# timsu1104/Open-vocabulary-3D-Object-Detection

Hardware: AMD Instinct MI355X
Metric: scenes/sec (train step) SUN RGB-D 20k pts nqueries=128 (higher is better)
Workload: dtype bf16; 1 GPU; SUN RGB-D train step, bs=8/GPU, 20000 pts, nqueries=128, 3DETR 256-d enc3/dec8, text-emb 640, AdamW + clip 0.1; global_batch=8, points=20000, parallelism=dp1

## Files before the change

include/ov3d.h:

```cpp
#ifndef OV3D_H_
#define OV3D_H_

#include <stdint.h>

#ifdef __cplusplus
extern "C" {
#endif

#define OV3D_OK 0
#define OV3D_EINVAL (-1)
#define OV3D_ELAUNCH (-2)

const char* ov3d_version(void);

int ov3d_fps(const float* xyz, int B, int N, int M, int32_t* idx_out, float* new_xyz_out,
             float* workspace, void* stream);
long long ov3d_fps_workspace(int B, int N);
int ov3d_fps_pair_status(const float* workspace, int B, int N, int M, int32_t* status,
                         void* stream);

int ov3d_nbr_max_fwd(const void* y, long long P, int S, int C, void* out, uint8_t* arg,
                     void* stream);
int ov3d_nbr_max_bwd(const void* g, const uint8_t* arg, long long P, int S, int C, void* dy,
                     void* stream);
// ... 234 lines not shown
                      const float* be2, float eps, const void* W1, long long ldw1, const void* b1,
                      float pf, int site_ffn, const void* W2, long long ldw2, const void* b2,
                      int k_quarters, float* s1, float* mean, float* rstd, void* x2, void* h,
                      void* y2, void* stream);
int ov3d_enc_post_bwd(int R, const float* ds1, const void* dy2, const float* s1, const float* mean,
                      const float* rstd, const void* h, const float* g2, const void* Wo,
                      long long ldwo, const void* W1, long long ldw1, const void* W2,
                      long long ldw2, float p1, const int64_t* seed, int site1, float pf,
                      int k_quarters, float* ds, void* dy1, void* dout, void* d1, float* partials,
                      int nparts, void* stream);

int ov3d_attn_fwd(const void* q, const void* k, const void* v, long long sq, long long sk,
                  long long sv, int B, int H, int Lq, int Lk, float scale, float dropout_p,
                  const int64_t* seed, int site, void* o, long long so, float* lse,
                  uint32_t* dropbits, float* workspace, int nsplit, void* stream);
long long ov3d_attn_fwd_workspace(int B, int H, int Lq, int Lk, int nsplit);
long long ov3d_attn_dropbits_words(int B, int H, int Lq, int Lk);
int ov3d_attn_bwd(const void* q, const void* k, const void* v, long long sq, long long sk,
                  long long sv, const void* o, long long so, const void* dout, long long sdo,
                  const float* lse, int B, int H, int Lq, int Lk, float scale, float dropout_p,
                  const uint32_t* dropbits, float* dvec, void* dq, long long sdq, void* dk,
                  long long sdk, void* dv, long long sdv, float* workspace, int nsplit,
                  void* stream);

typedef struct {
    const void* q; long long sq; const void* k; long long sk; const void* v; long long sv;
    const void* dout; long long sdo; const float* lse; const float* dvec;
    const uint32_t* dropbits; void* dk; long long sdk; void* dv; long long sdv;
} ov3d_attn_dkdv_job;
int ov3d_attn_bwd_dkdv_batch(const ov3d_attn_dkdv_job* jobs, int njobs, int B, int H, int Lq,
                             int Lk, float scale, float dropout_p, void* stream);

int ov3d_attn_small_bwd(int on);

long long ov3d_attn_maskbits_words(int B, int Lq, int Lk);
int ov3d_attn_mask_pack(const void* src, int kind, float thr, int B, int Lq, int Lk,
                        uint32_t* words, void* stream);
int ov3d_attn_fwd_masked(const void* q, const void* k, const void* v, long long sq, long long sk,
                         long long sv, int B, int H, int Lq, int Lk, float scale, float dropout_p,
                         const int64_t* seed, int site, void* o, long long so, float* lse,
                         uint32_t* dropbits, float* workspace, int nsplit,
                         const uint32_t* maskbits, void* stream);
int ov3d_attn_fwd_pregen(const void* q, const void* k, const void* v, long long sq, long long sk,
                         long long sv, int B, int H, int Lq, int Lk, float scale, float dropout_p,
                         const int64_t* seed, int site, void* o, long long so, float* lse,
                         uint32_t* dropbits, float* workspace, int nsplit, const uint32_t* maskbits,
                         void* stream);
int ov3d_attn_dropgen(int B, int H, int Lq, int Lk, float dropout_p, const int64_t* seed, int site,
                      uint32_t* dropbits, void* stream);
int ov3d_attn_bwd_masked(const void* q, const void* k, const void* v, long long sq, long long sk,
                         long long sv, const void* o, long long so, const void* dout, long long sdo,
                         const float* lse, int B, int H, int Lq, int Lk, float scale,
                         float dropout_p, const uint32_t* dropbits, float* dvec, void* dq,
                         long long sdq, void* dk, long long sdk, void* dv, long long sdv,
                         float* workspace, int nsplit, const uint32_t* maskbits, void* stream);

int ov3d_wgrad(const void* dy, long long ldy, const void* x, long long ldx, int R, int N, int K,
               float* dW, long long ldw, float* db, float* workspace, int* counters, int nsplit,
               void* stream);
int ov3d_wgrad_bn(const void* dy, long long ldy, const void* x, long long ldx, int R, int N, int K,
                  const float* scale, const float* shift, float* dW, long long ldw, float* db,
                  float* workspace, int* counters, int nsplit, void* stream);
long long ov3d_wgrad_workspace(int R, int N, int K, int nsplit);
typedef struct {
    const void* dy; long long ldy; const void* x; long long ldx;
    int R, N, K, nsplit;
// ... 277 lines not shown
```

open-vocabulary-3d-object-detection_amd/csrc/attn.hip:

```cpp
#include <math.h>
#include <type_traits>
#include <stdlib.h>

#include "common.h"

namespace {

typedef __bf16 bf16;
typedef __bf16 bf16x8 __attribute__((ext_vector_type(8)));
typedef __bf16 bf16x4 __attribute__((ext_vector_type(4)));
typedef float f32x16 __attribute__((ext_vector_type(16)));
typedef short s16x4 __attribute__((ext_vector_type(4)));
typedef float f32x2 __attribute__((ext_vector_type(2)));
typedef __bf16 bf16x2 __attribute__((ext_vector_type(2)));
typedef uint32_t u32x4 __attribute__((ext_vector_type(4)));
typedef short s16x2 __attribute__((ext_vector_type(2)));

constexpr int D = 64;
constexpr int KB = 64;
constexpr int QW = 32;
constexpr int LDK = 72;

__device__ __forceinline__ int isw(int r) { return (((r >> 1) & 1) << 2) | ((r >> 2) & 3); }
__device__ __forceinline__ int img(int r, int c) { return r * D + 8 * ((c >> 3) ^ isw(r)) + (c & 7); }
// ... 96 lines not shown
    return fmaxf(__builtin_bit_cast(float, (uint32_t)r[0]), __builtin_bit_cast(float, (uint32_t)r[1]));
}

__device__ __forceinline__ bf16x8 prescale8(bf16x8 v, float c) {
    bf16x8 r;
#pragma unroll
    for (int j = 0; j < 8; ++j) r[j] = (bf16)((float)v[j] * c);
    return r;
}

__device__ __forceinline__ bf16x8 kslots(float x0, float x1, bool on) {
    bf16x8 r;
#pragma unroll
    for (int j = 0; j < 8; ++j) r[j] = (bf16)0.f;
    if (on) {
        r[0] = (bf16)x0;
        r[1] = (bf16)x1;
    }
    return r;
}
__device__ __forceinline__ float bf16_hi(float x) { return (float)(bf16)x; }
__device__ __forceinline__ float bf16_lo(float x) {
    return __builtin_isinf(x) ? 0.f : x - bf16_hi(x);
}

constexpr float kStabBig = 32768.f;
__device__ __forceinline__ float stabiliser(float x) {
    const float hi = bf16_hi(x);
    return fabsf(x) < kStabBig ? hi : hi + bf16_hi(bf16_lo(x));
}

constexpr float RESCALE_THR = 8.f;

constexpr int kMaxCombine = 16;

#ifdef OV3D_ATTN_PROBE
__device__ unsigned long long* g_attn_probe;
#define PROBE_ENTRY const unsigned long long pr_entry = __builtin_amdgcn_s_memtime();
#define PROBE_DECL unsigned long long pr_t = __builtin_amdgcn_s_memtime(), pr_acc[8] = {0, 0, 0, 0, 0, 0, 0, 0}; \
    pr_acc[7] = pr_t - pr_entry;
#define PROBE(i) do { const unsigned long long t_ = __builtin_amdgcn_s_memtime(); pr_acc[i] += t_ - pr_t; pr_t = t_; } while (0)
#define PROBE_END do { if ((threadIdx.x & 63) == 0 && g_attn_probe) { \
    unsigned long long* o_ = g_attn_probe + (((size_t)blockIdx.z * gridDim.y + blockIdx.y) * gridDim.x + blockIdx.x) * 32 + (threadIdx.x >> 6) * 8; \
    for (int i_ = 0; i_ < 8; ++i_) o_[i_] = pr_acc[i_]; } } while (0)
#else
#define PROBE_ENTRY
#define PROBE_DECL
#define PROBE(i) do { } while (0)
#define PROBE_END do { } while (0)
#endif

__device__ __forceinline__ f32x16 mfma(bf16x8 a, bf16x8 b, f32x16 c) {
    return __builtin_amdgcn_mfma_f32_32x32x16_bf16(a, b, c, 0, 0, 0);
}

__device__ __forceinline__ bf16x4 tr16(const bf16* p) {
    s16x4 r = __builtin_amdgcn_ds_read_tr16_b64_v4i16(
        (__attribute__((address_space(3))) s16x4*)(p));
    return __builtin_bit_cast(bf16x4, r);
}

__device__ __forceinline__ bf16x8 v_operand(const bf16* Vs, int lane, int dt, int t, int s) {
    const int g = lane >> 4, i = lane & 15;
    const int d0 = 32 * dt + 16 * (g & 1) + 4 * (i & 3);
    const int k0 = 32 * t + 16 * s + 4 * (g >> 1) + (i >> 2);
    const bf16x4 lo = tr16(Vs + img(k0, d0));
// ... 36 lines not shown
    const int tid = threadIdx.x, lane = tid & 63, wave = tid >> 6;
    const int r = lane & 31, h = lane >> 5;
    int bx, bh;
    xcd_block(bx, bh);
    const int q0 = bx * (4 * QW) + wave * QW;
    if (q0 >= a.Lq) return;
    const uint32_t qh = drop_query_base(drop_head_mix(a.seed, a.site, bh), q0 + r) +
                        (uint32_t)(2 * h) * kPairMul;
    uint32_t* const wq_lane = a.wq + ((size_t)bh * a.Lq + q0 + r) * 2 + h;
    const size_t wq_tile = (size_t)gridDim.y * a.Lq * 2;
    uint32_t* const wk_lane = a.wk + ((size_t)(q0 >> 5) * gridDim.y + bh) * ((size_t)a.nkt * 64) +
                              drop_key(r, h);
    const short ts = (short)((int)a.thresh - 32768);
    const s16x2 tsig = {ts, ts};
    const int per = (a.nkt + gridDim.z - 1) / gridDim.z;
    const int kt1 = min(a.nkt, (int)(blockIdx.z + 1) * per);
    for (int kt = blockIdx.z * per; kt < kt1; ++kt) {
        const uint32_t hb = qh + (uint32_t)(32 * kt) * kPairMul;
        uint32_t dw = 0;
#pragma unroll
        for (int t = 0; t < 2; ++t)
#pragma unroll
            for (int i = 0; i < 16; i += 2) {
                const uint32_t c = 16 * t + ((i & 3) >> 1) + 4 * (i >> 2);
                const uint32_t dm = drop_halves(drop_mix(hb + c * kPairMul), tsig);
                const int jb = 8 * t + (i >> 1);
                dw |= dm & ((1u << jb) | (1u << (16 + jb)));
            }
        wq_lane[(size_t)kt * wq_tile] = dw;
        wk_lane[64 * kt] = transpose32(dw, r);
    }
}

template <bool DROP, bool MASK, bool BITS>
__device__ __forceinline__ void attn_fwd_body(const AttnArgs& a) {
    PROBE_ENTRY
    __shared__ __attribute__((aligned(16))) bf16 KVs[2][2][KB * LDK];
    bf16 (*const Ks)[KB * LDK] = KVs[0];
    bf16 (*const Vs)[KB * LDK] = KVs[1];
    const int tid = threadIdx.x, lane = tid & 63, wave = tid >> 6;
    const int r = lane & 31, h = lane >> 5;
    int bx, bh;
    xcd_block(bx, bh);
    const int b = bh / a.H, hh = bh - b * a.H;
    const int q0 = bx * (4 * QW) + wave * QW;
    const bool active = q0 < a.Lq;
    const int kbeg = blockIdx.z * a.keys_per_split;
    const int kend = min(a.Lk, kbeg + a.keys_per_split);

    bf16x8 qf[4];
    {
        const int qi = active ? q0 + r : 0;
        const bf16* qrow = a.q + ((size_t)qi * a.B + b) * a.sq + hh * D;
#pragma unroll
        for (int s = 0; s < 4; ++s)
            qf[s] = prescale8(*reinterpret_cast<const bf16x8*>(qrow + 16 * s + 8 * h), a.scale2);
    }
    uint32_t qh = 0;
    if (DROP && !BITS) qh = drop_query_base(drop_head_mix(a.seed, a.site, bh), active ? q0 + r : 0) +
                            (uint32_t)(2 * h) * kPairMul;
    uint32_t* const wq_lane = DROP ? a.wq + ((size_t)bh * a.Lq + (active ? q0 + r : 0)) * 2 + h : nullptr;
    const size_t wq_tile = (size_t)gridDim.y * a.Lq * 2;
    uint32_t* const wk_lane = (DROP && !BITS) ? a.wk + ((size_t)(q0 >> 5) * gridDim.y + bh) * ((size_t)a.nkt * 64) +
                                         drop_key(r, h) : nullptr;
    uint32_t dw_prev = 0;
    uint32_t dw_cur = 0, dw_next = 0;
    uint32_t mw_cur = 0, mw_next = 0;
    const uint32_t* const mrow = MASK ? a.mq + ((size_t)b * a.Lq + (active ? q0 + r : 0)) * 2 + h : nullptr;
    const size_t mtile = (size_t)a.B * a.Lq * 2;
    auto store_drop = [&](int kbp) {
        wq_lane[(size_t)(kbp >> 6) * wq_tile] = dw_prev;
        wk_lane[kbp] = transpose32(dw_prev, r);
// ... 17 lines not shown
            const int key = kb + (tid >> 3) + 32 * c;
            size_t ko = k0off + (size_t)(kb + 32 * c) * rowk, vo = v0off + (size_t)(kb + 32 * c) * rowv;
            if (key >= a.Lk) {
                ko -= (size_t)(key - (a.Lk - 1)) * rowk;
                vo -= (size_t)(key - (a.Lk - 1)) * rowv;
            }
            kr[c] = *reinterpret_cast<const bf16x8*>(a.k + ko);
            vr[c] = *reinterpret_cast<const bf16x8*>(a.v + vo);
        }
    };
    auto store = [&](int buf) {
#pragma unroll
        for (int c = 0; c < 2; ++c) {
            const int idx = tid + 256 * c, key = idx >> 3, ch = idx & 7;
            *reinterpret_cast<bf16x8*>(&Ks[buf][img(key, 8 * ch)]) = kr[c];
            *reinterpret_cast<bf16x8*>(&Vs[buf][img(key, 8 * ch)]) = vr[c];
        }
    };

    f32x16 o[2];
#pragma unroll
    for (int i = 0; i < 16; ++i) o[0][i] = o[1][i] = 0.f;
    float mb = 0.f;
    bool unset = true;
    const bf16x8 k1 = kslots(1.f, 1.f, h == 0);
    bf16x8 kmb = kslots(0.f, 0.f, false);
    f32x16 lacc;
#pragma unroll
    for (int i = 0; i < 16; ++i) lacc[i] = 0.f;
    bf16x8 ones;
#pragma unroll
    for (int j = 0; j < 8; ++j) ones[j] = (bf16)1.f;

    if (kbeg < kend) {
        load(kbeg);
        store(0);
        if (DROP && BITS && active) dw_cur = wq_lane[(size_t)(kbeg >> 6) * wq_tile];
        if (MASK && active) mw_cur = mrow[(size_t)(kbeg >> 6) * mtile];
    }
    __syncthreads();
    PROBE_DECL
    int buf = 0;
    for (int kb = kbeg; kb < kend; kb += KB, buf ^= 1) {
        const bool more = kb + KB < kend;
        PROBE(0);
        {
            const bf16* K = Ks[buf];
            const bf16* V = Vs[buf];
            if (MASK && more) mw_next = mrow[(size_t)((kb >> 6) + 1) * mtile];
            const uint32_t mw = mw_cur;
            if (DROP && BITS && more) dw_next = wq_lane[(size_t)((kb >> 6) + 1) * wq_tile];
            const uint32_t kwin = ~dw_cur;
            bf16x8 ka[2][4];
#pragma unroll
            for (int t = 0; t < 2; ++t)
#pragma unroll
                for (int s = 0; s < 4; ++s)
                    ka[t][s] = *reinterpret_cast<const bf16x8*>(K + img(32 * t + r, 16 * s + 8 * h));
            f32x16 st[2];
#pragma unroll
            for (int t = 0; t < 2; ++t) {
#pragma unroll
                for (int i = 0; i < 16; ++i)
                    st[t][i] = MASK ? __builtin_bit_cast(float, bit_mask(mw, score_bit(t, i)) & 0xFF800000u) : 0.f;
                st[t] = mfma(k1, kmb, st[t]);
            }
#pragma unroll
            for (int s = 0; s < 4; ++s)
#pragma unroll
                for (int t = 0; t < 2; ++t) st[t] = mfma(ka[t][s], qf[s], st[t]);
            bf16x8 va[2][2][2];
#pragma unroll
            for (int dt = 0; dt < 2; ++dt)
#pragma unroll
                for (int t = 0; t < 2; ++t)
#pragma unroll
                    for (int s = 0; s < 2; ++s) va[dt][t][s] = v_operand(V, lane, dt, t, s);
            if (more) load(kb + KB);
            if (DROP && !BITS && kb > kbeg && active) store_drop(kb - KB);
            PROBE(1);
            const int nvalid = kend - kb;
            if (nvalid < KB) {
#pragma unroll
                for (int t = 0; t < 2; ++t)
#pragma unroll
                    for (int i = 0; i < 16; ++i)
                        if (32 * t + (i & 3) + 8 * (i >> 2) + 4 * h >= nvalid) st[t][i] = -INFINITY;
            }
            float mx = -INFINITY;
#pragma unroll
            for (int t = 0; t < 2; ++t)
#pragma unroll
                for (int i = 0; i < 16; ++i) mx = fmaxf(mx, st[t][i]);
            mx = max_halves(mx);
            PROBE(2);
            const bool seen = mx > -INFINITY;
            if (__any(mx > RESCALE_THR || (unset && seen))) {
                const float mn = (mx > 0.f || (unset && seen)) ? stabiliser(mb + mx) : mb;
                const float d = mn - mb;
                const float alpha = unset ? 1.f : fast_exp2(-d);
                lacc[0] *= alpha;
#pragma unroll
                for (int i = 0; i < 16; ++i) {
                    o[0][i] *= alpha;
                    o[1][i] *= alpha;
                }
#pragma unroll
                for (int t = 0; t < 2; ++t)
#pragma unroll
                    for (int i = 0; i < 16; ++i) st[t][i] -= d;
                mb = mn;
// ... 16 lines not shown
#endif
                    uint32_t pk = pack_bf16(p0, p1);
                    praw[t][i >> 3][(i & 7) >> 1] = pk;
                    if (DROP && BITS) {
                        const int jb = 8 * t + (i >> 1);
                        const s16x2 kh = __builtin_bit_cast(s16x2, kwin << (15 - jb));
                        pk &= __builtin_bit_cast(uint32_t, (s16x2)(kh >> (s16x2){15, 15}));
                    } else if (DROP) {
                        const uint32_t c = 16 * t + ((i & 3) >> 1) + 4 * (i >> 2);
                        const uint32_t dm = drop_halves(drop_mix(hb + c * kPairMul), tsig);
                        pk &= ~dm;
                        const int jb = 8 * t + (i >> 1);
                        dw |= dm & ((1u << jb) | (1u << (16 + jb)));
                    }
                    pw[t][i >> 3][(i & 7) >> 1] = pk;
                }
            if (DROP && !BITS) dw_prev = dw;
            if (DROP && BITS) dw_cur = dw_next;
            if (MASK) mw_cur = mw_next;
            PROBE(3);
#pragma unroll
            for (int t = 0; t < 2; ++t)
#pragma unroll
                for (int s = 0; s < 2; ++s) {
                    const bf16x8 pf = __builtin_bit_cast(bf16x8, pw[t][s]);
#pragma unroll
                    for (int dt = 0; dt < 2; ++dt) o[dt] = mfma(va[dt][t][s], pf, o[dt]);
#ifndef OV3D_ATTN_VALU_ROWSUM
                    lacc = mfma(ones, __builtin_bit_cast(bf16x8, praw[t][s]), lacc);
#endif
                }
        }
        PROBE(4);
        if (more) store(buf ^ 1);
        PROBE(5);
        __syncthreads();
        PROBE(6);
    }
    PROBE_END;
    if (active && DROP && !BITS && kend > kbeg) store_drop((kend - 1) & ~(KB - 1));
#ifdef OV3D_ATTN_VALU_ROWSUM
    const float ltot = l + __shfl_xor(l, 32);
#else
    const float ltot = lacc[0];
#endif
    const int q = q0 + r;
    const int ql = wave * QW + r;
    if (a.nsplit == 1) {
        const float inv = ltot > 0.f ? a.keep_scale / ltot : 0.f;
        bf16* const so = &KVs[0][0][0];
#pragma unroll
        for (int dt = 0; dt < 2; ++dt)
#pragma unroll
            for (int g = 0; g < 4; ++g) {
                bf16x4 w;
#pragma unroll
                for (int j = 0; j < 4; ++j) w[j] = (bf16)(o[dt][4 * g + j] * inv);
                *reinterpret_cast<bf16x4*>(so + ql * LDK + 32 * dt + 8 * g + 4 * h) = w;
            }
        if (active && h == 0) a.lse[(size_t)bh * a.Lq + q] = mb + log2f(ltot);
        __syncthreads();
#pragma unroll
        for (int i = 0; i < 4; ++i) {
            const int c = tid + 256 * i, row = c >> 3, d8 = (c & 7) * 8;
            const int qq = bx * (4 * QW) + row;
            if (qq < a.Lq)
                *reinterpret_cast<bf16x8*>(a.o + ((size_t)qq * a.B + b) * a.so + hh * D + d8) =
                    *reinterpret_cast<const bf16x8*>(so + row * LDK + d8);
        }
    } else {
        constexpr int LDF = D + 4;
        float* const sf = reinterpret_cast<float*>(&KVs[0][0][0]);
        static_assert(sizeof(KVs) >= 128 * LDF * sizeof(float), "fp32 staging rows overrun KVs");
#pragma unroll
        for (int dt = 0; dt < 2; ++dt)
#pragma unroll
            for (int g = 0; g < 4; ++g)
                *reinterpret_cast<float4*>(sf + ql * LDF + 32 * dt + 8 * g + 4 * h) =
                    make_float4(o[dt][4 * g] * a.keep_scale, o[dt][4 * g + 1] * a.keep_scale,
                                o[dt][4 * g + 2] * a.keep_scale, o[dt][4 * g + 3] * a.keep_scale);
        const size_t rbase = ((size_t)blockIdx.z * gridDim.y + bh) * a.Lq;
        if (active && h == 0) {
            a.part_ml[2 * (rbase + q)] = ltot > 0.f ? mb : -INFINITY;
            a.part_ml[2 * (rbase + q) + 1] = ltot;
        }
        __syncthreads();
#pragma unroll
        for (int i = 0; i < 8; ++i) {
            const int c = tid + 256 * i, row = c >> 4, d4 = (c & 15) * 4;
            const int qq = bx * (4 * QW) + row;
            if (qq < a.Lq)
                *reinterpret_cast<float4*>(a.part_o + (rbase + qq) * D + d4) =
                    *reinterpret_cast<const float4*>(sf + row * LDF + d4);
        }
    }
}

template <bool DROP, bool MASK, bool BITS>
__global__ void __launch_bounds__(256, 2) attn_fwd_kernel(AttnArgs a) {
    ov3d_stamp(a.stamp, 0);
    attn_fwd_body<DROP, MASK, BITS>(a);
    ov3d_stamp(a.stamp, 1);
}

template <int NS>
__global__ void __launch_bounds__(256) attn_combine_kernel(AttnArgs a) {
    const int w = (blockIdx.x * blockDim.x + threadIdx.x) >> 6, d = threadIdx.x & 63;
    const int BH = a.B * a.H;
    if (w >= BH * a.Lq) return;
    const int bh = w / a.Lq, q = w - bh * a.Lq;
    const int b = bh / a.H, hh = bh - b * a.H;
    float M = -INFINITY;
    float L = 0.f, acc = 0.f;
    if (a.nsplit <= NS) {
        float ms[NS], ls[NS], os[NS];
#pragma unroll
        for (int s = 0; s < NS; ++s) {
            const int sc = s < a.nsplit ? s : a.nsplit - 1;
            const size_t row = ((size_t)sc * BH + bh) * a.Lq + q;
            ms[s] = a.part_ml[2 * row];
            ls[s] = a.part_ml[2 * row + 1];
            os[s] = a.part_o[row * D + d];
        }
#pragma unroll
        for (int s = 0; s < NS; ++s)
            if (s >= a.nsplit) ms[s] = -INFINITY;
#pragma unroll
        for (int s = 0; s < NS; ++s) M = fmaxf(M, ms[s]);
#pragma unroll
        for (int s = 0; s < NS; ++s) {
            if (ms[s] == -INFINITY) continue;
            const float wgt = exp2f(ms[s] - M);
            L = fmaf(ls[s], wgt, L);
            acc = fmaf(os[s], wgt, acc);
// ... 240 lines not shown
template <bool DROP, bool MASK, bool RAGGED>
__global__ void __launch_bounds__(256, 2) attn_bwd_dq_kernel(AttnBwdArgs A) {
    ov3d_stamp(A.f.stamp, 0);
    attn_bwd_dq_body<DROP, MASK, RAGGED>(A);
    ov3d_stamp(A.f.stamp, 1);
}

__global__ void __launch_bounds__(256) attn_dq_combine_kernel(AttnBwdArgs A) {
    const AttnArgs& a = A.f;
    const int BH = a.B * a.H;
    const long long t = (long long)blockIdx.x * blockDim.x + threadIdx.x;
    if (t >= (long long)BH * a.Lq * (D / 4)) return;
    const int d4 = (int)(t % (D / 4));
    const long long w = t / (D / 4);
    const int bh = (int)(w / a.Lq), q = (int)(w - (long long)bh * a.Lq);
    const int b = bh / a.H, hh = bh - b * a.H;
    float4 acc = make_float4(0.f, 0.f, 0.f, 0.f);
    for (int sp = 0; sp < a.nsplit; ++sp) {
        const float4 v = *reinterpret_cast<const float4*>(
            a.part_o + (((size_t)sp * BH + bh) * a.Lq + q) * D + 4 * d4);
        acc.x += v.x;
        acc.y += v.y;
        acc.z += v.z;
        acc.w += v.w;
    }
    bf16x4 o;
    o[0] = (bf16)(acc.x * A.scale);
    o[1] = (bf16)(acc.y * A.scale);
    o[2] = (bf16)(acc.z * A.scale);
    o[3] = (bf16)(acc.w * A.scale);
    *reinterpret_cast<bf16x4*>(A.dq + ((size_t)q * a.B + b) * A.sdq + hh * D + 4 * d4) = o;
}

template <bool DROP, bool MASK, bool OWN_D = false>
__device__ __forceinline__ void attn_bwd_dkdv_body(const AttnBwdArgs& A) {
    const AttnArgs& a = A.f;
    constexpr int QB = 64;
    __shared__ __attribute__((aligned(16))) bf16 Qs[2][QB * LDK];
    __shared__ __attribute__((aligned(16))) bf16 Ds[2][QB * LDK];
    __shared__ __attribute__((aligned(16))) float Ls[2][QB];
    __shared__ __attribute__((aligned(16))) float Dv[2][QB];
    const int tid = threadIdx.x, lane = tid & 63, wave = tid >> 6;
    const int r = lane & 31, h = lane >> 5;
    int bx, bh;
    xcd_block(bx, bh);
    const int b = bh / a.H, hh = bh - b * a.H;
    const int k0 = bx * (4 * 32) + wave * 32;
    const bool active = k0 < a.Lk;
    const int ki = active ? min(k0 + r, a.Lk - 1) : 0;
    const uint32_t* wcol = DROP ? a.wk + (size_t)bh * ((size_t)a.nkt * 64) + ki : nullptr;
    const size_t wstride = (size_t)gridDim.y * a.nkt * 64;
    uint32_t wn[2] = {0u, 0u};
    const uint32_t* mcol = MASK ? a.mk + (size_t)b * ((size_t)a.nkt * 64) + ki : nullptr;
    const size_t mstride = (size_t)a.B * a.nkt * 64;
    uint32_t mn[2] = {0u, 0u};

    bf16x8 kf[4], vf[4];
    {
        const bf16* krow = a.k + ((size_t)ki * a.B + b) * a.sk + hh * D;
        const bf16* vrow = a.v + ((size_t)ki * a.B + b) * a.sv + hh * D;
#pragma unroll
        for (int s = 0; s < 4; ++s) {
            kf[s] = prescale8(*reinterpret_cast<const bf16x8*>(krow + 16 * s + 8 * h), a.scale2);
            vf[s] = *reinterpret_cast<const bf16x8*>(vrow + 16 * s + 8 * h);
        }
    }

// ... 39 lines not shown
        if (MASK && active) {
#pragma unroll
            for (int u = 0; u < 2; ++u)
                mn[u] = qb + 32 * u < a.Lq ? mcol[(size_t)((qb >> 5) + u) * mstride] : 0u;
        }
    };
    auto store = [&](int buf) {
#pragma unroll
        for (int c = 0; c < 2; ++c) {
            const int idx = tid + 256 * c, qq = idx >> 3, ch = idx & 7;
            *reinterpret_cast<bf16x8*>(&Qs[buf][img(qq, 8 * ch)]) = qr[c];
            *reinterpret_cast<bf16x8*>(&Ds[buf][img(qq, 8 * ch)]) = dr[c];
        }
        if (tid < QB) {
            Ls[buf][tid] = lr;
            if (!OWN_D) Dv[buf][tid] = dvr;
        }
        if (OWN_D) {
#pragma unroll
            for (int c = 0; c < 2; ++c) {
                float t = 0.f;
#pragma unroll
                for (int j = 0; j < 8; ++j) t = fmaf((float)dr[c][j], (float)orr[c][j], t);
                t += __shfl_xor(t, 1);
                t += __shfl_xor(t, 2);
                t += __shfl_xor(t, 4);
                if ((tid & 7) == 0) Dv[buf][(tid >> 3) + 32 * c] = -t / a.keep_scale;
            }
        }
    };
    f32x16 dkt[2], dvt[2];
#pragma unroll
    for (int i = 0; i < 16; ++i) dkt[0][i] = dkt[1][i] = dvt[0][i] = dvt[1][i] = 0.f;
    load(0);
    store(0);
    uint32_t wc[2] = {wn[0], wn[1]};
    uint32_t mc[2] = {mn[0], mn[1]};
    __syncthreads();
    int buf = 0;
    for (int qb = 0; qb < a.Lq; qb += QB, buf ^= 1) {
        const bool more = qb + QB < a.Lq;
        if (more) load(qb + QB);
        {
            const bf16* Q = Qs[buf];
            const bf16* DO = Ds[buf];
#pragma unroll
            for (int u = 0; u < 2; ++u) {
                float lv[16], dv[16];
#pragma unroll
                for (int g = 0; g < 4; ++g) {
                    const int qrow = 32 * u + 8 * g + 4 * h;
                    const float4 l4 = *reinterpret_cast<const float4*>(&Ls[buf][qrow]);
                    const float4 d4 = *reinterpret_cast<const float4*>(&Dv[buf][qrow]);
                    lv[4 * g] = l4.x; lv[4 * g + 1] = l4.y; lv[4 * g + 2] = l4.z; lv[4 * g + 3] = l4.w;
                    dv[4 * g] = d4.x; dv[4 * g + 1] = d4.y; dv[4 * g + 2] = d4.z; dv[4 * g + 3] = d4.w;
                }
                const uint32_t msh = MASK ? mc[u] >> (4 * h) : 0u;
                f32x16 st, dpt;
#pragma unroll
                for (int i = 0; i < 16; ++i) {
                    st[i] = MASK ? neg_inf_if(lv[i], msh, 8 * (i >> 2) + (i & 3)) : lv[i];
                    dpt[i] = dv[i];
                }
#pragma unroll
                for (int s = 0; s < 4; ++s) {
                    const bf16x8 qa = *reinterpret_cast<const bf16x8*>(Q + img(32 * u + r, 16 * s + 8 * h));
                    const bf16x8 da = *reinterpret_cast<const bf16x8*>(DO + img(32 * u + r, 16 * s + 8 * h));
                    st = mfma(qa, kf[s], st);
                    dpt = mfma(da, vf[s], dpt);
                }
                const uint32_t ksh = DROP ? ~wc[u] >> (4 * h) : 0u;
                u32x4 pw[2], dsw[2];
#pragma unroll
                for (int g = 0; g < 4; ++g) {
                    float pd[4], ds[4];
#pragma unroll
                    for (int j = 0; j < 4; ++j) {
                        const int i = 4 * g + j;
                        const float p = fast_exp2(st[i]);
                        float pk = p, dp = dpt[i];
                        if (DROP) {
                            const uint32_t km = bit_mask(ksh, 8 * g + j);
                            pk = __builtin_bit_cast(float, __builtin_bit_cast(uint32_t, p) & km);
                            dp = __builtin_bit_cast(float, (__builtin_bit_cast(uint32_t, dp) & km) |
                                                               (__builtin_bit_cast(uint32_t, dv[i]) & ~km));
                        }
                        pd[j] = pk;
                        ds[j] = p * dp;
                    }
                    pw[g >> 1][2 * (g & 1)] = pack_bf16(pd[0], pd[1]);
                    pw[g >> 1][2 * (g & 1) + 1] = pack_bf16(pd[2], pd[3]);
                    dsw[g >> 1][2 * (g & 1)] = pack_bf16(ds[0], ds[1]);
                    dsw[g >> 1][2 * (g & 1) + 1] = pack_bf16(ds[2], ds[3]);
                }
#pragma unroll
                for (int dt = 0; dt < 2; ++dt)
#pragma unroll
                    for (int s = 0; s < 2; ++s) {
                        const int tt = u;
                        dvt[dt] = mfma(v_operand(DO, lane, dt, tt, s), __builtin_bit_cast(bf16x8, pw[s]), dvt[dt]);
                        dkt[dt] = mfma(v_operand(Q, lane, dt, tt, s), __builtin_bit_cast(bf16x8, dsw[s]), dkt[dt]);
                    }
            }
        }
        if (more) store(buf ^ 1);
        wc[0] = wn[0];
        wc[1] = wn[1];
        mc[0] = mn[0];
        mc[1] = mn[1];
        __syncthreads();
    }
    bf16* const sk = &Qs[0][0];
    bf16* const sv = &Ds[0][0];
    const int kl = wave * 32 + r;
#pragma unroll
    for (int dt = 0; dt < 2; ++dt)
#pragma unroll
        for (int g = 0; g < 4; ++g) {
            bf16x4 wk, wv;
#pragma unroll
            for (int j = 0; j < 4; ++j) {
                wk[j] = (bf16)(dkt[dt][4 * g + j] * (A.scale * a.keep_scale));
                wv[j] = (bf16)(dvt[dt][4 * g + j] * a.keep_scale);
            }
            *reinterpret_cast<bf16x4*>(sk + kl * LDK + 32 * dt + 8 * g + 4 * h) = wk;
            *reinterpret_cast<bf16x4*>(sv + kl * LDK + 32 * dt + 8 * g + 4 * h) = wv;
        }
    __syncthreads();
#pragma unroll
    for (int i = 0; i < 4; ++i) {
        const int c = tid + 256 * i, row = c >> 3, d8 = (c & 7) * 8;
        const int key = bx * 128 + row;
        if (key < a.Lk) {
            *reinterpret_cast<bf16x8*>(A.dk + ((size_t)key * a.B + b) * A.sdk + hh * D + d8) =
                *reinterpret_cast<const bf16x8*>(sk + row * LDK + d8);
            *reinterpret_cast<bf16x8*>(A.dv + ((size_t)key * a.B + b) * A.sdv + hh * D + d8) =
                *reinterpret_cast<const bf16x8*>(sv + row * LDK + d8);
        }
    }
}

template <bool DROP, bool MASK>
__global__ void __launch_bounds__(256, 2) attn_bwd_dkdv_kernel(AttnBwdArgs A) {
    ov3d_stamp(A.stamp2, 0);
    attn_bwd_dkdv_body<DROP, MASK>(A);
    ov3d_stamp(A.stamp2, 1);
}

template <bool DROP, bool RAGGED>
__global__ void __launch_bounds__(256, 2) attn_bwd_small_kernel(AttnBwdArgs A) {
    attn_bwd_dq_body<DROP, false, RAGGED>(A);
    __syncthreads();
    attn_bwd_dkdv_body<DROP, false>(A);
}

template <bool DROP, bool RAGGED>
__global__ void __launch_bounds__(256, 2) attn_bwd_small2_kernel(AttnBwdArgs A) {
    if (blockIdx.z == 0) attn_bwd_dq_body<DROP, false, RAGGED>(A);
    else attn_bwd_dkdv_body<DROP, false, true>(A);
}

constexpr int kDkdvBatchMax = 8;
struct AttnBwdBatch {
    AttnBwdArgs a[kDkdvBatchMax];
};
static_assert(sizeof(AttnBwdBatch) <= 4000, "kernel argument space");

template <bool DROP>
__global__ void __launch_bounds__(256, 2) attn_bwd_dkdv_batch_kernel(AttnBwdBatch g) {
    attn_bwd_dkdv_body<DROP, false>(g.a[blockIdx.z]);
}

template <int KIND>
__device__ __forceinline__ bool masked_value(float v, float thr) {
    if (KIND == 2) v = sqrtf(fmaxf(v, 0.f));
    return v >= thr;
}

__device__ __forceinline__ float point_sqdist(const float4 pq, const float4 pk) {
    float acc = 0.f;
    acc = fmaf(-2.f * pq.x, pk.x, acc);
    acc = fmaf(-2.f * pq.y, pk.y, acc);
    acc = fmaf(-2.f * pq.z, pk.z, acc);
    acc = fmaf(pq.w, 1.f, acc);
    acc = fmaf(1.f, pk.w, acc);
    return acc;
}

template <int KIND>
__device__ __forceinline__ bool mask_at(const void* src, size_t e, float thr, int Lk = 0) {
    if (KIND == 0) return ((const uint8_t*)src)[e] != 0;
    if (KIND == 3) {
        const size_t bq = e / (size_t)Lk, k = e - bq * (size_t)Lk, b = bq / (size_t)Lk;
        const float4* pts = (const float4*)src;
        return point_sqdist(pts[bq], pts[b * Lk + k]) >= thr;
    }
    return masked_value<KIND>(((const float*)src)[e], thr);
}

template <int KIND>
__global__ void __launch_bounds__(256) attn_mask_pack_kernel(const void* __restrict__ src, float thr,
                                                             int B, int Lq, int Lk, int nkt,
                                                             uint32_t* __restrict__ words) {
// ... 115 lines not shown
    words[W + u] = w;
}

}

extern "C" long long ov3d_attn_dropbits_words(int B, int H, int Lq, int Lk) {
    if (B <= 0 || H <= 0 || Lq <= 0 || Lk <= 0 || (Lq % QW)) return 0;
    return 4LL * ((Lk + KB - 1) / KB) * B * H * Lq;
}

static void set_dropbits(AttnArgs& a, uint32_t* bits) {
    a.nkt = (a.Lk + KB - 1) / KB;
    a.wq = bits;
    a.wk = bits ? bits + 2 * (size_t)a.nkt * a.B * a.H * a.Lq : nullptr;
}

static bool small_bwd_split() {
    const char* e = getenv("OV3D_ATTN_SMALL_SPLIT");
    return !(e && e[0] == '0');
}

static int g_small_bwd = -1;
static bool fuse_small_bwd() {
    if (g_small_bwd < 0) {
        const char* e = getenv("OV3D_ATTN_SMALL_BWD");
        g_small_bwd = (e && e[0] == '0') ? 0 : 1;
    }
    return g_small_bwd != 0;
}

extern "C" int ov3d_attn_small_bwd(int on) {
    const int prev = fuse_small_bwd() ? 1 : 0;
    if (on >= 0) g_small_bwd = on ? 1 : 0;
    return prev;
}

constexpr int kDropgenSplit = 4;
static bool dropgen_ahead(int Lq, int Lk) {
    const char* e = getenv("OV3D_ATTN_DROPGEN_MIN");
    const long long min_pairs = e ? atoll(e) : -1;
    return min_pairs >= 0 && (long long)Lq * Lk >= min_pairs;
}

static void set_maskbits(AttnArgs& a, const uint32_t* bits) {
    a.mq = bits;
    a.mk = bits ? bits + 2 * (size_t)a.nkt * a.B * a.Lq : nullptr;
}

extern "C" long long ov3d_attn_maskbits_words(int B, int Lq, int Lk) {
    if (B <= 0 || Lq <= 0 || Lk <= 0 || (Lq % QW)) return 0;
    return 4LL * ((Lk + KB - 1) / KB) * B * Lq;
}

extern "C" int ov3d_attn_mask_pack(const void* src, int kind, float thr, int B, int Lq, int Lk,
                                   uint32_t* words, void* stream) {
    if (!src || !words || kind < 0 || kind > 3 || B <= 0 || Lq <= 0 || Lk <= 0 || (Lq % QW))
        return OV3D_EINVAL;
    if (kind == 3 && (Lq != Lk || ((uintptr_t)src & 15))) return OV3D_EINVAL;
    const int nkt = (Lk + KB - 1) / KB;
    const long long n = (long long)B * Lq * nkt + ov3d_attn_maskbits_words(B, Lq, Lk) / 2;
    hipStream_t st = ov3d_stream(stream);
    if (kind == 0)
        attn_mask_pack_kernel<0><<<ov3d_cdiv(n, 256), 256, 0, st>>>(src, thr, B, Lq, Lk, nkt, words);
    else if (kind == 1)
        attn_mask_pack_kernel<1><<<ov3d_cdiv(n, 256), 256, 0, st>>>(src, thr, B, Lq, Lk, nkt, words);
    else if (kind == 2)
// ... 82 lines not shown
    a.v = (const bf16*)v;
    a.sq = sq;
    a.sk = sk;
    a.sv = sv;
    a.B = B;
    a.H = H;
    a.Lq = Lq;
    a.Lk = Lk;
    a.scale2 = scale * 1.4426950408889634f;
    a.thresh = dropout_p > 0.f ? (uint32_t)fminf(rintf(dropout_p * 65536.0f), 65535.0f) : 0u;
    a.keep_scale = 1.f / (1.f - dropout_p);
    a.seed = seed;
    a.site = (uint32_t)site;
    a.o = (bf16*)o;
    a.so = so;
    a.lse = lse;
    int kps = (Lk + nsplit - 1) / nsplit;
    kps = (kps + KB - 1) / KB * KB;
    nsplit = (Lk + kps - 1) / kps;
    a.keys_per_split = kps;
    a.nsplit = nsplit;
    a.part_o = workspace;
    a.part_ml = workspace ? workspace + (size_t)nsplit * B * H * Lq * D : nullptr;
    set_dropbits(a, dropbits);
    set_maskbits(a, maskbits);
    hipStream_t st = ov3d_stream(stream);
    dim3 grid((Lq + 4 * QW - 1) / (4 * QW), B * H, nsplit);
    a.stamp = ov3d_stamp_take(0, (long long)Lq * Lk, (long long)grid.x * grid.y * grid.z * 4);
    const bool bits = a.thresh && (pregen || dropgen_ahead(Lq, Lk));
    if (bits && !pregen) {
        attn_dropgen_kernel<<<dim3(grid.x, grid.y, min(a.nkt, kDropgenSplit)), 256, 0, st>>>(a);
        OV3D_LAUNCH_CHECK();
    }
    if (maskbits) {
        if (bits)
            attn_fwd_kernel<true, true, true><<<grid, 256, 0, st>>>(a);
        else if (a.thresh)
            attn_fwd_kernel<true, true, false><<<grid, 256, 0, st>>>(a);
        else
            attn_fwd_kernel<false, true, false><<<grid, 256, 0, st>>>(a);
    } else if (bits) {
        attn_fwd_kernel<true, false, true><<<grid, 256, 0, st>>>(a);
    } else if (a.thresh) {
        attn_fwd_kernel<true, false, false><<<grid, 256, 0, st>>>(a);
    } else {
        attn_fwd_kernel<false, false, false><<<grid, 256, 0, st>>>(a);
    }
    OV3D_LAUNCH_CHECK();
    if (nsplit > 1) {
        const long long waves = (long long)B * H * Lq;
        const int nb = ov3d_cdiv(waves * 64, 256);
        if (nsplit <= 2) attn_combine_kernel<2><<<nb, 256, 0, st>>>(a);
        else if (nsplit <= 4) attn_combine_kernel<4><<<nb, 256, 0, st>>>(a);
        else if (nsplit <= 8) attn_combine_kernel<8><<<nb, 256, 0, st>>>(a);
        else attn_combine_kernel<kMaxCombine><<<nb, 256, 0, st>>>(a);
        OV3D_LAUNCH_CHECK();
    }
    return OV3D_OK;
}

extern "C" int ov3d_attn_fwd_masked(const void* q, const void* k, const void* v, long long sq,
                                    long long sk, long long sv, int B, int H, int Lq, int Lk,
                                    float scale, float dropout_p, const int64_t* seed, int site,
                                    void* o, long long so, float* lse, uint32_t* dropbits,
                                    float* workspace, int nsplit, const uint32_t* maskbits,
                                    void* stream) {
    return attn_fwd_impl(q, k, v, sq, sk, sv, B, H, Lq, Lk, scale, dropout_p, seed, site, o, so, lse,
// ... 199 lines not shown
            a.B = B;
            a.H = H;
            a.Lq = Lq;
            a.Lk = Lk;
            a.scale2 = scale * 1.4426950408889634f;
            a.thresh = dropout_p > 0.f ? (uint32_t)fminf(rintf(dropout_p * 65536.0f), 65535.0f) : 0u;
            a.keep_scale = 1.f / (1.f - dropout_p);
            a.seed = nullptr;
            a.site = 0;
            a.o = nullptr;
            a.so = 0;
            a.lse = (float*)J.lse;
            a.part_o = nullptr;
            a.part_ml = nullptr;
            a.nsplit = 1;
            a.keys_per_split = Lk;
            set_dropbits(a, (uint32_t*)J.dropbits);
            set_maskbits(a, nullptr);
            A.o = nullptr;
            A.dout = (const bf16*)J.dout;
            A.sdo = J.sdo;
            A.dvec = (float*)J.dvec;
            A.dq = nullptr;
            A.dk = (bf16*)J.dk;
            A.dv = (bf16*)J.dv;
            A.sdq = 0;
            A.sdk = J.sdk;
            A.sdv = J.sdv;
            A.scale = scale;
            a.stamp = nullptr;
            A.stamp2 = nullptr;
        }
        const dim3 gk((Lk + 127) / 128, B * H, n);
        if (dropout_p > 0.f)
            attn_bwd_dkdv_batch_kernel<true><<<gk, 256, 0, st>>>(g);
        else
            attn_bwd_dkdv_batch_kernel<false><<<gk, 256, 0, st>>>(g);
        OV3D_LAUNCH_CHECK();
    }
    return OV3D_OK;
}
```

Before: 1777 scenes/s.

## Preload all K/V or Q/dO tiles up front for short attention sequences

Adds a SHORT variant of the forward attention kernel. When a split holds at most four key tiles and the grid fits in one round of CUs, it issues all K/V global loads up front into registers, stages them into a larger shared-memory buffer, and drops the per-tile double-buffer loads and barriers. A matching DEEP variant of the batched dK/dV backward kernel preloads both Q/dO tiles, plus lse, dvec and dropout words, when Lq<=128. This removes serial load-then-sync latency in short loops, at the cost of more registers and shared memory, which may lower occupancy. Both paths are on by default and can be switched off through an env var or API mask.

Result: no change. 1786 scenes/s (median of 6 runs) (+0.5%).

```diff
diff --git a/include/ov3d.h b/include/ov3d.h
--- a/include/ov3d.h
+++ b/include/ov3d.h
@@ -290,6 +290,8 @@
                              int Lk, float scale, float dropout_p, void* stream);
 
 int ov3d_attn_small_bwd(int on);
+
+int ov3d_attn_deep(int mask);
 
 long long ov3d_attn_maskbits_words(int B, int Lq, int Lk);
 int ov3d_attn_mask_pack(const void* src, int kind, float thr, int B, int Lq, int Lk,
diff --git a/open-vocabulary-3d-object-detection_amd/csrc/attn.hip b/open-vocabulary-3d-object-detection_amd/csrc/attn.hip
--- a/open-vocabulary-3d-object-detection_amd/csrc/attn.hip
+++ b/open-vocabulary-3d-object-detection_amd/csrc/attn.hip
@@ -152,6 +152,8 @@
 
 constexpr float RESCALE_THR = 8.f;
 
+constexpr int kShortTiles = 4;
+
 constexpr int kMaxCombine = 16;
 
 #ifdef OV3D_ATTN_PROBE
@@ -254,12 +256,14 @@
     }
 }
 
-template <bool DROP, bool MASK, bool BITS>
+template <bool DROP, bool MASK, bool BITS, bool SHORT = false>
 __device__ __forceinline__ void attn_fwd_body(const AttnArgs& a) {
     PROBE_ENTRY
-    __shared__ __attribute__((aligned(16))) bf16 KVs[2][2][KB * LDK];
-    bf16 (*const Ks)[KB * LDK] = KVs[0];
-    bf16 (*const Vs)[KB * LDK] = KVs[1];
+    constexpr int NIMG = SHORT ? kShortTiles : 2;
+    constexpr int IMG = SHORT ? KB * D : KB * LDK;
+    __shared__ __attribute__((aligned(16))) bf16 KVs[2][NIMG][IMG];
+    bf16 (*const Ks)[IMG] = KVs[0];
+    bf16 (*const Vs)[IMG] = KVs[1];
     const int tid = threadIdx.x, lane = tid & 63, wave = tid >> 6;
     const int r = lane & 31, h = lane >> 5;
     int bx, bh;
@@ -343,7 +347,32 @@
 #pragma unroll
     for (int j = 0; j < 8; ++j) ones[j] = (bf16)1.f;
 
-    if (kbeg < kend) {
+    bf16x8 krs[SHORT ? kShortTiles : 1][2], vrs[SHORT ? kShortTiles : 1][2];
+    auto store_short = [&](int t) {
+#pragma unroll
+        for (int c = 0; c < 2; ++c) {
+            const int idx = tid + 256 * c, key = idx >> 3, ch = idx & 7;
+            *reinterpret_cast<bf16x8*>(&Ks[t][img(key, 8 * ch)]) = krs[SHORT ? t : 0][c];
+            *reinterpret_cast<bf16x8*>(&Vs[t][img(key, 8 * ch)]) = vrs[SHORT ? t : 0][c];
+        }
+    };
+    if constexpr (SHORT) {
+        const size_t kcol = (size_t)b * a.sk + hh * D + 8 * (tid & 7);
+        const size_t vcol = (size_t)b * a.sv + hh * D + 8 * (tid & 7);
+#pragma unroll
+        for (int t = 0; t < kShortTiles; ++t) {
+#pragma unroll
+            for (int c = 0; c < 2; ++c) {
+                const int key = min(kbeg + KB * t + 32 * c + (tid >> 3), kend - 1);
+                krs[t][c] = *reinterpret_cast<const bf16x8*>(a.k + kcol + (size_t)key * rowk);
+                vrs[t][c] = *reinterpret_cast<const bf16x8*>(a.v + vcol + (size_t)key * rowv);
+            }
+            if (t & 1) __builtin_amdgcn_sched_barrier(0);
+        }
+        if (DROP && BITS) dw_cur = wq_lane[(size_t)(kbeg >> 6) * wq_tile];
+        store_short(0);
+        store_short(1);
+    } else if (kbeg < kend) {
         load(kbeg);
         store(0);
         if (DROP && BITS && active) dw_cur = wq_lane[(size_t)(kbeg >> 6) * wq_tile];
@@ -352,8 +381,15 @@
     __syncthreads();
     PROBE_DECL
     int buf = 0;
-    for (int kb = kbeg; kb < kend; kb += KB, buf ^= 1) {
+    for (int kb = kbeg; kb < kend; kb += KB, buf = SHORT ? buf + 1 : buf ^ 1) {
         const bool more = kb + KB < kend;
+        if constexpr (SHORT) {
+            if (buf == 2) {
+                store_short(2);
+                store_short(3);
+                __syncthreads();
+            }
+        }
         PROBE(0);
         {
             const bf16* K = Ks[buf];
@@ -387,7 +423,7 @@
                 for (int t = 0; t < 2; ++t)
 #pragma unroll
                     for (int s = 0; s < 2; ++s) va[dt][t][s] = v_operand(V, lane, dt, t, s);
-            if (more) load(kb + KB);
+            if (!SHORT && more) load(kb + KB);
             if (DROP && !BITS && kb > kbeg && active) store_drop(kb - KB);
             PROBE(1);
             const int nvalid = kend - kb;
@@ -470,12 +506,13 @@
                 }
         }
         PROBE(4);
-        if (more) store(buf ^ 1);
+        if (!SHORT && more) store(buf ^ 1);
         PROBE(5);
-        __syncthreads();
+        if (!SHORT) __syncthreads();
         PROBE(6);
     }
     PROBE_END;
+    if (SHORT) __syncthreads();
     if (active && DROP && !BITS && kend > kbeg) store_drop((kend - 1) & ~(KB - 1));
 #ifdef OV3D_ATTN_VALU_ROWSUM
     const float ltot = l + __shfl_xor(l, 32);
@@ -538,6 +575,13 @@
 __global__ void __launch_bounds__(256, 2) attn_fwd_kernel(AttnArgs a) {
     ov3d_stamp(a.stamp, 0);
     attn_fwd_body<DROP, MASK, BITS>(a);
+    ov3d_stamp(a.stamp, 1);
+}
+
+template <bool DROP, bool BITS>
+__global__ void __launch_bounds__(256, 2) attn_fwd_short_kernel(AttnArgs a) {
+    ov3d_stamp(a.stamp, 0);
+    attn_fwd_body<DROP, false, BITS, true>(a);
     ov3d_stamp(a.stamp, 1);
 }
 
@@ -844,7 +888,7 @@
     *reinterpret_cast<bf16x4*>(A.dq + ((size_t)q * a.B + b) * A.sdq + hh * D + 4 * d4) = o;
 }
 
-template <bool DROP, bool MASK, bool OWN_D = false>
+template <bool DROP, bool MASK, bool OWN_D = false, bool DEEP = false>
 __device__ __forceinline__ void attn_bwd_dkdv_body(const AttnBwdArgs& A) {
     const AttnArgs& a = A.f;
     constexpr int QB = 64;
@@ -950,15 +994,64 @@
     f32x16 dkt[2], dvt[2];
 #pragma unroll
     for (int i = 0; i < 16; ++i) dkt[0][i] = dkt[1][i] = dvt[0][i] = dvt[1][i] = 0.f;
-    load(0);
-    store(0);
-    uint32_t wc[2] = {wn[0], wn[1]};
-    uint32_t mc[2] = {mn[0], mn[1]};
+    uint32_t wc[2], mc[2];
+    if constexpr (DEEP) {
+        static_assert(!OWN_D && !MASK, "the deep dK / dV loads: D from dvec, no mask");
+        bf16x8 qs[2][2], ds[2][2];
+        float ls[2], dvs[2];
+        uint32_t ws[2][2];
+        const size_t qcol = (size_t)b * a.sq + hh * D + 8 * (tid & 7);
+        const size_t dcol = (size_t)b * A.sdo + hh * D + 8 * (tid & 7);
+        const int nqb = a.Lq >> 5;
+#pragma unroll
+        for (int u = 0; u < 2; ++u) {
+#pragma unroll
+            for (int c = 0; c < 2; ++c) {
+                const int qq = min(QB * u + 32 * c + (tid >> 3), a.Lq - 1);
+                qs[u][c] = *reinterpret_cast<const bf16x8*>(a.q + qcol + (size_t)qq * rowq);
+                ds[u][c] = *reinterpret_cast<const bf16x8*>(A.dout + dcol + (size_t)qq * rowd);
+            }
+            const int qc = min(QB * u + (tid & (QB - 1)), a.Lq - 1);
+            ls[u] = a.lse[(size_t)bh * a.Lq + qc];
+            dvs[u] = A.dvec[(size_t)bh * a.Lq + qc];
+            if (DROP) {
+#pragma unroll
+                for (int v = 0; v < 2; ++v)
+                    ws[u][v] = wcol[(size_t)min(2 * u + v, nqb - 1) * wstride];
+            }
+        }
+#pragma unroll
+        for (int u = 0; u < 2; ++u) {
+#pragma unroll
+            for (int c = 0; c < 2; ++c) {
+                const int idx = tid + 256 * c, qq = idx >> 3, ch = idx & 7;
+                *reinterpret_cast<bf16x8*>(&Qs[u][img(qq, 8 * ch)]) = qs[u][c];
+                *reinterpret_cast<bf16x8*>(&Ds[u][img(qq, 8 * ch)]) = ds[u][c];
+            }
+            if (tid < QB) {
+                Ls[u][tid] = -(QB * u + tid < a.Lq ? ls[u] : INFINITY);
+                Dv[u][tid] = -dvs[u] / a.keep_scale;
+            }
+        }
+#pragma unroll
+        for (int v = 0; v < 2; ++v) {
+            wc[v] = (DROP && active && 32 * v < a.Lq) ? ws[0][v] : 0u;
+            wn[v] = (DROP && active && QB + 32 * v < a.Lq) ? ws[1][v] : 0u;
+            mc[v] = 0u;
+        }
+    } else {
+        load(0);
+        store(0);
+        wc[0] = wn[0];
+        wc[1] = wn[1];
+        mc[0] = mn[0];
+        mc[1] = mn[1];
+    }
     __syncthreads();
     int buf = 0;
     for (int qb = 0; qb < a.Lq; qb += QB, buf ^= 1) {
         const bool more = qb + QB < a.Lq;
-        if (more) load(qb + QB);
+        if (!DEEP && more) load(qb + QB);
         {
             const bf16* Q = Qs[buf];
             const bf16* DO = Ds[buf];
@@ -1021,13 +1114,14 @@
                     }
             }
         }
-        if (more) store(buf ^ 1);
+        if (!DEEP && more) store(buf ^ 1);
         wc[0] = wn[0];
         wc[1] = wn[1];
         mc[0] = mn[0];
         mc[1] = mn[1];
-        __syncthreads();
-    }
+        if (!DEEP) __syncthreads();
+    }
+    if (DEEP) __syncthreads();
     bf16* const sk = &Qs[0][0];
     bf16* const sv = &Ds[0][0];
     const int kl = wave * 32 + r;
@@ -1084,9 +1178,9 @@
 };
 static_assert(sizeof(AttnBwdBatch) <= 4000, "kernel argument space");
 
-template <bool DROP>
+template <bool DROP, bool DEEP>
 __global__ void __launch_bounds__(256, 2) attn_bwd_dkdv_batch_kernel(AttnBwdBatch g) {
-    attn_bwd_dkdv_body<DROP, false>(g.a[blockIdx.z]);
+    attn_bwd_dkdv_body<DROP, false, false, DEEP>(g.a[blockIdx.z]);
 }
 
 template <int KIND>
@@ -1268,6 +1362,34 @@
 extern "C" int ov3d_attn_small_bwd(int on) {
     const int prev = fuse_small_bwd() ? 1 : 0;
     if (on >= 0) g_small_bwd = on ? 1 : 0;
+    return prev;
+}
+
+constexpr int kDeepDefault = 3;
+static int g_deep = -1;
+static int deep_mask() {
+    if (g_deep < 0) {
+        const char* e = getenv("OV3D_ATTN_DEEP");
+        g_deep = e && e[0] ? (atoi(e) & 3) : kDeepDefault;
+    }
+    return g_deep;
+}
+
+static bool one_round(long long workgroups) {
+    static int cus = 0;
+    if (!cus) {
+        int dev = 0, n = 0;
+        if (hipGetDevice(&dev) != hipSuccess ||
+            hipDeviceGetAttribute(&n, hipDeviceAttributeMultiprocessorCount, dev) != hipSuccess || n <= 0)
+            n = 256;
+        cus = n;
+    }
+    return workgroups <= cus;
+}
+
+extern "C" int ov3d_attn_deep(int mask) {
+    const int prev = deep_mask();
+    if (mask >= 0) g_deep = mask & 3;
     return prev;
 }
 
@@ -1416,7 +1538,15 @@
         attn_dropgen_kernel<<<dim3(grid.x, grid.y, min(a.nkt, kDropgenSplit)), 256, 0, st>>>(a);
         OV3D_LAUNCH_CHECK();
     }
-    if (maskbits) {
+    if (!maskbits && kps <= kShortTiles * KB && (deep_mask() & 1) &&
+        one_round((long long)grid.x * grid.y * grid.z)) {
+        if (bits)
+            attn_fwd_short_kernel<true, true><<<grid, 256, 0, st>>>(a);
+        else if (a.thresh)
+            attn_fwd_short_kernel<true, false><<<grid, 256, 0, st>>>(a);
+        else
+            attn_fwd_short_kernel<false, false><<<grid, 256, 0, st>>>(a);
+    } else if (maskbits) {
         if (bits)
             attn_fwd_kernel<true, true, true><<<grid, 256, 0, st>>>(a);
         else if (a.thresh)
@@ -1682,10 +1812,15 @@
             A.stamp2 = nullptr;
         }
         const dim3 gk((Lk + 127) / 128, B * H, n);
-        if (dropout_p > 0.f)
-            attn_bwd_dkdv_batch_kernel<true><<<gk, 256, 0, st>>>(g);
+        if (Lq <= 128 && (deep_mask() & 2)) {
+            if (dropout_p > 0.f)
+                attn_bwd_dkdv_batch_kernel<true, true><<<gk, 256, 0, st>>>(g);
+            else
+                attn_bwd_dkdv_batch_kernel<false, true><<<gk, 256, 0, st>>>(g);
+        } else if (dropout_p > 0.f)
+            attn_bwd_dkdv_batch_kernel<true, false><<<gk, 256, 0, st>>>(g);
         else
-            attn_bwd_dkdv_batch_kernel<false><<<gk, 256, 0, st>>>(g);
+            attn_bwd_dkdv_batch_kernel<false, false><<<gk, 256, 0, st>>>(g);
         OV3D_LAUNCH_CHECK();
     }
     return OV3D_OK;
```
